# debbiemarkslab/EVcouplings

Measured on NVIDIA H100. Metric: PLM gradient evals/s as N*L^2*q cell-ops/s, higher is better.
Workload: dtype f32 parameters/accumulation; tensor-core products as bf16 hi+lo pairs (16 mantissa bits)

## Files before the change

evcouplings_b200/csrc/api.cu:

```cuda
#include "../../include/evcplm.h"

#include <stdlib.h>

#include <algorithm>
#include <new>
#include <string>
#include <vector>

#include "common.cuh"
#include "internal.h"

namespace evc {
static thread_local std::string g_err;
void set_error(const std::string &msg) { g_err = msg; }
}

using namespace evc;

static cudaStream_t as_stream(void *s) { return reinterpret_cast<cudaStream_t>(s); }

static const char SUPPORTED_Q[] =
    "supported: 2 <= q <= 32 states with the gap as a state, 2 <= q <= 31 with the ignored gap coded q; "
    "every code must be below 32, the 5 bit-planes of the Hamming pass";

// ... 392 lines not shown

int evc_plm_eval_data(evc_plm_t *h, const float *d_x, float *d_g, double *d_fx, void *stream)
{
    if (!h || !d_x || !d_g || !d_fx) { set_error("evc_plm_eval_data: null pointer"); return 1; }
    cudaStream_t st = as_stream(stream);
    const PlmGeom &g = h->g;
    const bool prof = h->profiling;
    const bool tc = h->bwd_mode == 1;
    const bool tcf = h->fwd_mode == 1;
    const bool tcff = h->fwd_mode == 2;
    const int single = h->precision == 1 ? 1 : 0;
    void *rt_lo = single ? nullptr : h->d_rt_lo;
    float *gJ = d_g + (int64_t)g.L * g.q;
    if (tc && h->tc.n_chunks > 1) {
        if (!tcf) {
            set_error("evc_plm_eval_data: sequence chunks need the tensor-core forward (evc_plm_set_forward 1)");
            return 1;
        }
        h->ev_valid = false;
        if (plm_tcf_expand(g, h->tcf, d_x, h->d_wt_hi, h->d_wt_lo, single, st)) return 1;
        for (int c = 0; c < h->tc.n_chunks; c++) {
            const int64_t n0 = (int64_t)c * h->tc.C, nreal = std::min(h->tc.C, g.N - n0);
            if (plm_tcf_build_xsp(g, h->tcf, h->d_msa4, h->d_x1h, n0, st)) return 1;
            if (plm_tc_build_xt(g, h->tc, h->d_msa4, h->d_xt, n0, st)) return 1;
            if (plm_tcf_logits(g, h->tcf, h->tcf_maps, h->d_x1h, h->d_zt, single, nreal, st)) return 1;
            if (plm_tcf_softmax(g, h->tcf, h->d_zt, d_x, h->d_msa4, h->d_wts, h->d_rt_hi, rt_lo, h->tc.Kp,
                                h->d_gh_part2, h->d_fx_part2, n0, nreal, st))
                return 1;
            if (plm_tc_backward(g, h->tc, h->tc_maps, h->d_Gd, single, c, st)) return 1;
        }
        if (plm_tc_finalize_pairs(g, h->tc, h->d_Gd, h->tc.planes, gJ, 1.0f, st)) return 1;
        return plm_finalize_fields_n(g, h->d_gh_part2, h->d_fx_part2, d_g, d_fx, h->tcf.ntiles_s, st);
    }
    if (!tc || (!tcf && !tcff)) {
        if (require_gather_q(h, "evc_plm_eval_data") || ensure_gather(h)) return 1;
    }
    if (prof) EVC_CUDA(cudaEventRecord(h->ev[0], st));
    if (tcff) {
        if (plm_tcff_expand(g, h->tcff, d_x, h->d_wp_hi, h->d_wp_lo, single, st)) return 1;
        if (prof) EVC_CUDA(cudaEventRecord(h->ev[1], st));
        if (plm_tcff_forward(g, h->tcff, h->tcff_maps, d_x, h->d_msa4, h->d_wts, h->d_rt_hi, h->d_rt_lo, h->tc.Kp,
                             h->d_gh_part3, h->d_fx_part3, single, st))
            return 1;
        if (prof) {
            EVC_CUDA(cudaEventRecord(h->ev[2], st));
            EVC_CUDA(cudaEventRecord(h->ev[3], st));
        }
// ... 45 lines not shown

int evc_plm_set_backward(evc_plm_t *h, int32_t mode)
{
    if (!h) { set_error("evc_plm_set_backward: null handle"); return 1; }
    if (mode != 0 && mode != 1) { set_error("evc_plm_set_backward: mode must be 0 (gather) or 1 (tensor core)"); return 1; }
    if (mode == 0 && require_gather_q(h, "evc_plm_set_backward")) return 1;
    EVC_CUDA(cudaSetDevice(h->device));
    if (mode == 1 && !h->d_xt) {
        int sm_count = 0;
        EVC_CUDA(cudaDeviceGetAttribute(&sm_count, cudaDevAttrMultiProcessorCount, h->device));
        plm_tc_geometry(h->g, sm_count, h->seq_chunk, h->tc);
        const PlmTcGeom &t = h->tc;
        const TcBwdBytes b(t);
        if (!dalloc(h, &h->d_xt, b.xt) || !dalloc(h, &h->d_rt_hi, b.rt) || !dalloc(h, &h->d_rt_lo, b.rt) ||
            !dalloc(h, &h->d_Gd, b.gd)) {
            set_error(std::string("evc_plm_set_backward: device allocation failed: ") +
                      cudaGetErrorString(cudaGetLastError()));
            return 1;
        }
        EVC_CUDA(cudaMemset(h->d_xt, 0, b.xt));
        EVC_CUDA(cudaMemset(h->d_rt_hi, 0, b.rt));
        EVC_CUDA(cudaMemset(h->d_rt_lo, 0, b.rt));
        EVC_CUDA(cudaMemset(h->d_Gd, 0, b.gd));
        if (t.n_chunks == 1 && plm_tc_build_xt(h->g, t, h->d_msa4, h->d_xt, 0, 0)) return 1;
        EVC_CUDA(cudaDeviceSynchronize());
        h->tc_maps = aligned_alloc(64, round_up((int64_t)plm_tc_map_bytes(), 64));
        if (!h->tc_maps) { set_error("evc_plm_set_backward: out of host memory"); return 1; }
        if (plm_tc_make_maps(t, h->d_xt, h->d_rt_hi, h->d_rt_lo, h->tc_maps)) return 1;
    }
    h->bwd_mode = mode;
    return 0;
}

int evc_plm_set_forward(evc_plm_t *h, int32_t mode)
{
    if (!h) { set_error("evc_plm_set_forward: null handle"); return 1; }
    if (mode < 0 || mode > 2) {
        set_error("evc_plm_set_forward: mode must be 0 (gather), 1 (tensor core) or 2 (tensor core, fused softmax)");
        return 1;
    }
    if (mode == 0 && require_gather_q(h, "evc_plm_set_forward")) return 1;
    EVC_CUDA(cudaSetDevice(h->device));
    const int64_t chunk = plm_seq_chunk_round(h->seq_chunk);
    const bool chunked = chunk > 0 && chunk < h->g.N;
    if (mode == 2 && (!plm_tcff_supported(h->g) || (int64_t)h->g.L * h->g.q > 8192 || chunked)) mode = 1;
    if (mode >= 1) {
        if (evc_plm_set_backward(h, 1)) return 1;
        if (!h->d_x1h) {
            plm_tcf_geometry(h->g, h->tc, h->tcf);
            const PlmTcfGeom &t = h->tcf;
            const TcFwdBytes b(h->g, t);
// ... 204 lines not shown
            set_error("evc_plm_eval_host: device allocation failed");
            return 1;
        }
    }
    EVC_CUDA(cudaMemcpyAsync(h->d_x_tmp, x, nb, cudaMemcpyHostToDevice, 0));
    if (evc_plm_eval_data(h, h->d_x_tmp, h->d_g_tmp, h->d_fx_tmp, nullptr)) return 1;
    if (evc_plm_add_regulariser(h, h->d_x_tmp, h->d_g_tmp, h->d_fx_tmp, lambda_h, lambda_J, nullptr)) return 1;
    EVC_CUDA(cudaMemcpyAsync(gout, h->d_g_tmp, nb, cudaMemcpyDeviceToHost, 0));
    EVC_CUDA(cudaMemcpyAsync(fx_out, h->d_fx_tmp, 2 * sizeof(double), cudaMemcpyDeviceToHost, 0));
    EVC_CUDA(cudaStreamSynchronize(0));
    return 0;
}

int evc_plm_weighted_counts(evc_plm_t *h, float *d_fi_counts, float *d_fij_counts, void *stream)
{
    if (!h || !d_fi_counts || !d_fij_counts) { set_error("evc_plm_weighted_counts: null pointer"); return 1; }
    cudaStream_t st = as_stream(stream);
    const PlmGeom &g = h->g;
    if (h->bwd_mode == 1 && h->d_gh_part2) {
        const int ntiles = h->tcf.ntiles_s;
        const PlmTcGeom &t = h->tc;
        for (int c = 0; c < t.n_chunks; c++) {
            const int64_t n0 = (int64_t)c * t.C, nreal = std::min(t.C, g.N - n0);
            if (t.n_chunks > 1 && plm_tc_build_xt(g, t, h->d_msa4, h->d_xt, n0, st)) return 1;
            if (plm_tc_onehot_residual(g, ntiles, h->d_msa4, h->d_wts, h->d_rt_hi, h->d_rt_lo, t.Kp, h->d_gh_part2,
                                       h->d_fx_part2, n0, nreal, st))
                return 1;
            if (plm_tc_backward(g, t, h->tc_maps, h->d_Gd, 0, c, st)) return 1;
        }
        if (plm_tc_finalize_pairs(g, t, h->d_Gd, t.planes, d_fij_counts, 0.5f, st)) return 1;
        return plm_finalize_fields_n(g, h->d_gh_part2, nullptr, d_fi_counts, nullptr, ntiles, st);
    }
    if (require_gather_q(h, "evc_plm_weighted_counts") || ensure_gather(h)) return 1;
    EVC_CUDA(cudaMemsetAsync(h->d_G, 0, (size_t)g.w_floats() * sizeof(float), st));
    if (plm_onehot_residual(g, h->d_msa4, h->d_wts, h->d_R, h->d_gh_part, st)) return 1;
    if (plm_backward(g, h->d_R, h->d_perm, h->d_bstart, h->d_G, st)) return 1;
    return plm_finalize(g, h->d_G, h->d_gh_part, nullptr, d_fi_counts, d_fij_counts, nullptr, 0.5f, st);
}

int evc_ec_scores(const float *d_J_tri, const float *d_fij_tri, const float *d_fi, int32_t L, int32_t q,
                  float *d_fn_raw, float *d_fn_zero_sum, float *d_mi, void *stream)
{
    if (!d_J_tri) { set_error("evc_ec_scores: null pointer"); return 1; }
    return ec_scores(d_J_tri, d_fij_tri, d_fi, L, q, d_fn_raw, d_fn_zero_sum, d_mi, as_stream(stream));
}

int evc_plm_energies(evc_plm_t *h, const float *d_x, double *d_out, void *stream)
// ... 75 lines not shown
```

evcouplings_b200/csrc/internal.h:

```cpp
#pragma once
#include <cuda_runtime.h>
#include <stdint.h>

namespace evc {

int64_t hamming_plane_words(int64_t N, int L);
int64_t hamming_num_tiles(int64_t N);
int hamming_pack(const uint8_t *d_codes, int64_t N, int L, uint32_t *d_planes, cudaStream_t st);
int hamming_count_tiles(const uint32_t *d_planes, const int *d_mult, int64_t N, int L, int min_identical,
                        int64_t tile_begin, int64_t tile_end, int *d_counts, cudaStream_t st);

int identities_to_seq(const uint8_t *d_codes, const uint8_t *d_seq, int64_t N, int L, int *d_out, cudaStream_t st);

int msa_unique(const uint8_t *d_codes, int64_t N, int L, int *d_first, int *d_inverse, int *d_mult, int64_t *U_out,
               cudaStream_t st);

struct PlmGeom {
    int64_t N;
    int L;
    int Lp;
    int q;
    int QB;
    int S;
    int gap_code;
// ... 29 lines not shown
                 float *d_G, cudaStream_t st);
int plm_finalize(const PlmGeom &g, const float *d_G, const float *d_gh_part, const double *d_fx_part,
                 float *d_gh, float *d_gJ, double *d_fx, float scale_pair, cudaStream_t st);

constexpr int64_t PLM_SEQ_CHUNK_ALIGN = 768;
int64_t plm_seq_chunk_round(int64_t seq_chunk);
struct PlmTcGeom {
    int64_t C;
    int n_chunks;
    int64_t Mp;
    int64_t Np;
    int64_t Kp;
    int ksplit;
    int ksplit_last;
    int planes;
    int64_t kp_chunk(int c, int64_t N) const
    {
        const int64_t n = N - (int64_t)c * C < C ? N - (int64_t)c * C : C;
        return (n + 63) / 64 * 64;
    }
};
void plm_tc_geometry(const PlmGeom &g, int sm_count, int64_t seq_chunk, PlmTcGeom &t);
size_t plm_tc_map_bytes();
int plm_tc_build_xt(const PlmGeom &g, const PlmTcGeom &t, const uint32_t *d_msa4, void *d_xt, int64_t n0,
                    cudaStream_t st);
int plm_tc_make_maps(const PlmTcGeom &t, void *d_xt, void *d_rt_hi, void *d_rt_lo, void *maps_out_host);
int plm_tc_backward(const PlmGeom &g, const PlmTcGeom &t, const void *maps_host, float *d_Gd, int single, int chunk,
                    cudaStream_t st);
int plm_tc_onehot_residual(const PlmGeom &g, int ntiles, const uint32_t *d_msa4, const float *d_wts, void *d_rt_hi,
                           void *d_rt_lo, int64_t Kp, float *d_gh_part, double *d_fx_part, int64_t n0, int64_t nreal,
                           cudaStream_t st);
int plm_tc_finalize_pairs(const PlmGeom &g, const PlmTcGeom &t, const float *d_Gd, int planes, float *d_gJ,
                          float scale, cudaStream_t st);
struct PlmTcfGeom {
    int64_t Mp;
    int64_t Kw;
    int64_t Ns;
    int64_t Xrows;
    int ntiles_s;
};
void plm_tcf_geometry(const PlmGeom &g, const PlmTcGeom &tc, PlmTcfGeom &t);
int plm_tcf_build_x(const PlmGeom &g, const PlmTcfGeom &t, const uint32_t *d_msa4, void *d_x1h, int64_t n0,
                    cudaStream_t st);
int plm_tcf_build_xsp(const PlmGeom &g, const PlmTcfGeom &t, const uint32_t *d_msa4, void *d_x1h, int64_t n0,
                      cudaStream_t st);
int plm_tcf_make_maps(const PlmTcfGeom &t, void *d_wt_hi, void *d_wt_lo, void *maps_out_host);
int plm_tcf_expand(const PlmGeom &g, const PlmTcfGeom &t, const float *d_x, void *d_wt_hi, void *d_wt_lo,
                   int single, cudaStream_t st);
int plm_tcf_logits(const PlmGeom &g, const PlmTcfGeom &t, const void *maps_host, const void *d_x1h, float *d_zt,
// ... 111 lines not shown
```

evcouplings_b200/csrc/plm_tc.cu:

```cuda
#include <cuda.h>
#include <cuda_bf16.h>

#include <stdlib.h>

#include <algorithm>

#include "common.cuh"
#include "internal.h"

namespace evc {

constexpr int TC_BM = 128;
constexpr int TC_BN = 192;
constexpr int TC_BK = 64;
constexpr int TC_MAX_STAGES = 8;
constexpr int TC_A_BYTES = TC_BM * TC_BK * 2;
constexpr int TC_B_BYTES = TC_BN * TC_BK * 2;
constexpr int TC_SMEM_LIMIT = 232448;
constexpr int TC_SMEM_HEAD = 2048;
constexpr int TC_THREADS = 384;
constexpr int TC_CONSUMERS = 256;
constexpr int TC_K_CHUNK = 32;
constexpr int TC_MAX_KSPLIT = 8;
constexpr int TC_REG_PRODUCER = 40;
// ... 59 lines not shown

template <int R>
__device__ __forceinline__ void fence_regs(float *d)
{
#pragma unroll
    for (int i = 0; i < R; i++) asm volatile("" : "+f"(d[i])::"memory");
}

__device__ __forceinline__ void consumer_sync() { asm volatile("bar.sync 1, %0;" ::"n"(TC_CONSUMERS) : "memory"); }

__device__ __forceinline__ uint64_t make_desc_sw128(const void *smem_ptr)
{
    const uint32_t addr = smem_u32(smem_ptr);
    uint64_t d = 0;
    d |= (uint64_t)((addr >> 4) & 0x3FFF);
    d |= (uint64_t)1 << 16;
    d |= (uint64_t)(1024 >> 4) << 32;
    d |= (uint64_t)1 << 62;
    return d;
}

template <int N>
__device__ __forceinline__ void wgmma_bf16(float *d, uint64_t da, uint64_t db, uint32_t scale_d);
template <>
__device__ __forceinline__ void wgmma_bf16<192>(float *d, uint64_t da, uint64_t db, uint32_t scale_d)
{
    asm volatile(
        "{\n.reg .pred p;\n"
        "setp.ne.b32 p, %98, 0;\n"
        "wgmma.mma_async.sync.aligned.m64n192k16.f32.bf16.bf16 "
        "{"
        "%0, %1, %2, %3, %4, %5, %6, %7, %8, %9, %10, %11, %12, %13, %14, %15, "
        "%16, %17, %18, %19, %20, %21, %22, %23, %24, %25, %26, %27, %28, %29, %30, %31, "
        "%32, %33, %34, %35, %36, %37, %38, %39, %40, %41, %42, %43, %44, %45, %46, %47, "
        "%48, %49, %50, %51, %52, %53, %54, %55, %56, %57, %58, %59, %60, %61, %62, %63, "
        "%64, %65, %66, %67, %68, %69, %70, %71, %72, %73, %74, %75, %76, %77, %78, %79, "
        "%80, %81, %82, %83, %84, %85, %86, %87, %88, %89, %90, %91, %92, %93, %94, %95"
        "}, %96, %97, p, 1, 1, 0, 0;\n}\n"
        : "+f"(d[0]), "+f"(d[1]), "+f"(d[2]), "+f"(d[3]), "+f"(d[4]), "+f"(d[5]), "+f"(d[6]), "+f"(d[7]),
          "+f"(d[8]), "+f"(d[9]), "+f"(d[10]), "+f"(d[11]), "+f"(d[12]), "+f"(d[13]), "+f"(d[14]), "+f"(d[15]),
          "+f"(d[16]), "+f"(d[17]), "+f"(d[18]), "+f"(d[19]), "+f"(d[20]), "+f"(d[21]), "+f"(d[22]), "+f"(d[23]),
          "+f"(d[24]), "+f"(d[25]), "+f"(d[26]), "+f"(d[27]), "+f"(d[28]), "+f"(d[29]), "+f"(d[30]), "+f"(d[31]),
          "+f"(d[32]), "+f"(d[33]), "+f"(d[34]), "+f"(d[35]), "+f"(d[36]), "+f"(d[37]), "+f"(d[38]), "+f"(d[39]),
          "+f"(d[40]), "+f"(d[41]), "+f"(d[42]), "+f"(d[43]), "+f"(d[44]), "+f"(d[45]), "+f"(d[46]), "+f"(d[47]),
          "+f"(d[48]), "+f"(d[49]), "+f"(d[50]), "+f"(d[51]), "+f"(d[52]), "+f"(d[53]), "+f"(d[54]), "+f"(d[55]),
          "+f"(d[56]), "+f"(d[57]), "+f"(d[58]), "+f"(d[59]), "+f"(d[60]), "+f"(d[61]), "+f"(d[62]), "+f"(d[63]),
          "+f"(d[64]), "+f"(d[65]), "+f"(d[66]), "+f"(d[67]), "+f"(d[68]), "+f"(d[69]), "+f"(d[70]), "+f"(d[71]),
          "+f"(d[72]), "+f"(d[73]), "+f"(d[74]), "+f"(d[75]), "+f"(d[76]), "+f"(d[77]), "+f"(d[78]), "+f"(d[79]),
          "+f"(d[80]), "+f"(d[81]), "+f"(d[82]), "+f"(d[83]), "+f"(d[84]), "+f"(d[85]), "+f"(d[86]), "+f"(d[87]),
          "+f"(d[88]), "+f"(d[89]), "+f"(d[90]), "+f"(d[91]), "+f"(d[92]), "+f"(d[93]), "+f"(d[94]), "+f"(d[95])
        : "l"(da), "l"(db), "r"(scale_d));
}
template <>
__device__ __forceinline__ void wgmma_bf16<176>(float *d, uint64_t da, uint64_t db, uint32_t scale_d)
{
    asm volatile(
        "{\n.reg .pred p;\n"
        "setp.ne.b32 p, %90, 0;\n"
        "wgmma.mma_async.sync.aligned.m64n176k16.f32.bf16.bf16 "
        "{"
        "%0, %1, %2, %3, %4, %5, %6, %7, %8, %9, %10, %11, %12, %13, %14, %15, "
        "%16, %17, %18, %19, %20, %21, %22, %23, %24, %25, %26, %27, %28, %29, %30, %31, "
        "%32, %33, %34, %35, %36, %37, %38, %39, %40, %41, %42, %43, %44, %45, %46, %47, "
        "%48, %49, %50, %51, %52, %53, %54, %55, %56, %57, %58, %59, %60, %61, %62, %63, "
        "%64, %65, %66, %67, %68, %69, %70, %71, %72, %73, %74, %75, %76, %77, %78, %79, "
        "%80, %81, %82, %83, %84, %85, %86, %87"
        "}, %88, %89, p, 1, 1, 0, 0;\n}\n"
        : "+f"(d[0]), "+f"(d[1]), "+f"(d[2]), "+f"(d[3]), "+f"(d[4]), "+f"(d[5]), "+f"(d[6]), "+f"(d[7]),
          "+f"(d[8]), "+f"(d[9]), "+f"(d[10]), "+f"(d[11]), "+f"(d[12]), "+f"(d[13]), "+f"(d[14]), "+f"(d[15]),
          "+f"(d[16]), "+f"(d[17]), "+f"(d[18]), "+f"(d[19]), "+f"(d[20]), "+f"(d[21]), "+f"(d[22]), "+f"(d[23]),
          "+f"(d[24]), "+f"(d[25]), "+f"(d[26]), "+f"(d[27]), "+f"(d[28]), "+f"(d[29]), "+f"(d[30]), "+f"(d[31]),
          "+f"(d[32]), "+f"(d[33]), "+f"(d[34]), "+f"(d[35]), "+f"(d[36]), "+f"(d[37]), "+f"(d[38]), "+f"(d[39]),
          "+f"(d[40]), "+f"(d[41]), "+f"(d[42]), "+f"(d[43]), "+f"(d[44]), "+f"(d[45]), "+f"(d[46]), "+f"(d[47]),
          "+f"(d[48]), "+f"(d[49]), "+f"(d[50]), "+f"(d[51]), "+f"(d[52]), "+f"(d[53]), "+f"(d[54]), "+f"(d[55]),
// ... 127 lines not shown
};
__device__ __forceinline__ TcSmem tc_smem_layout(unsigned char *smem_dyn)
{
    unsigned char *base = reinterpret_cast<unsigned char *>((reinterpret_cast<uintptr_t>(smem_dyn) + 1023) &
                                                            ~static_cast<uintptr_t>(1023));
    TcSmem l;
    l.full = reinterpret_cast<uint64_t *>(base);
    l.empty = l.full + TC_MAX_STAGES;
    l.ring = base + 1024;
    return l;
}
__device__ __forceinline__ void tc_init_barriers(const TcSmem &l, int n_stages)
{
    if (threadIdx.x == 0) {
        for (int s = 0; s < n_stages; s++) {
            mbar_init(&l.full[s], 1);
            mbar_init(&l.empty[s], TC_CONSUMERS);
        }
        mbar_fence_init();
    }
    __syncthreads();
}

template <int SINGLE, int ACC = 0>
__global__ void __launch_bounds__(TC_THREADS, 1)
tc_gemm_kernel(const __grid_constant__ CUtensorMap tm0, const __grid_constant__ CUtensorMap tm1,
               const __grid_constant__ CUtensorMap tm2, float *__restrict__ D, int64_t ldd, int m_tiles, int n_tiles,
               int num_kb, int k_chunk, int mgroup, int n_stages, int ksplit, int64_t plane, int acc_planes)
{
    constexpr int BYTES0 = TC_A_BYTES;
    constexpr int BYTES1 = TC_B_BYTES;
    constexpr int BYTES2 = TC_B_BYTES;
    constexpr int stage_bytes = BYTES0 + BYTES1 + (SINGLE ? 0 : BYTES2);
    extern __shared__ unsigned char smem_dyn[];
    const TcSmem l = tc_smem_layout(smem_dyn);
    const int tiles = m_tiles * n_tiles;
    const int slice = (int)blockIdx.x / tiles;
    int m_tile, n_tile;
    decode_tile((int)blockIdx.x - slice * tiles, m_tiles, n_tiles, mgroup, m_tile, n_tile);
    const int kb_per = (num_kb + ksplit - 1) / ksplit;
    const int kb_begin = slice * kb_per, kb_end = min(num_kb, kb_begin + kb_per);
    tc_init_barriers(l, n_stages);

    if (threadIdx.x < 128) {
        setmaxnreg_dec<TC_REG_PRODUCER>();
        if (threadIdx.x == 0) {
            int s = 0;
            uint32_t ph = 0;
            for (int kb = kb_begin; kb < kb_end; kb++) {
                mbar_wait_bounded(&l.empty[s], ph ^ 1u);
                unsigned char *st = l.ring + s * stage_bytes;
                mbar_expect_tx(&l.full[s], (uint32_t)stage_bytes);
                tma_load_2d(st, &tm0, kb * TC_BK, m_tile * TC_BM, &l.full[s]);
                tma_load_2d(st + BYTES0, &tm1, kb * TC_BK, n_tile * TC_BN, &l.full[s]);
                if (!SINGLE) tma_load_2d(st + BYTES0 + BYTES1, &tm2, kb * TC_BK, n_tile * TC_BN, &l.full[s]);
                if (++s == n_stages) { s = 0; ph ^= 1u; }
            }
        }
    } else {
        setmaxnreg_inc<TC_REG_CONSUMER>();
        const int cw = (threadIdx.x >> 7) - 1;
        constexpr uint64_t OFF1 = (uint64_t)(BYTES0 >> 4), OFF2 = (uint64_t)((BYTES0 + BYTES1) >> 4);
        const uint64_t arow = (uint64_t)((cw * 64 * TC_BK * 2) >> 4);
        const uint64_t desc0 = make_desc_sw128(l.ring);
        float acc[TC_BN / 2], sum[TC_BN / 2];
#pragma unroll
        for (int u = 0; u < TC_BN / 2; u++) acc[u] = 0.f;
        const int n_chunks = (kb_end - kb_begin + k_chunk - 1) / k_chunk;
        int s = 0;
        uint32_t ph = 0;
        for (int c = 0; c < n_chunks; c++) {
            const int kb0 = kb_begin + c * k_chunk, kb1 = min(kb_end, kb0 + k_chunk);
            tc_mainloop<TC_BN>(acc, l.full, l.empty, s, ph, n_stages, stage_bytes, kb0, kb1, desc0,
                               arow, OFF1, arow, OFF2, !SINGLE);
#pragma unroll
            for (int u = 0; u < TC_BN / 2; u++) sum[u] = (c == 0) ? acc[u] : sum[u] + acc[u];
        }
        const int t = threadIdx.x & 127;
        const int64_t row = (int64_t)m_tile * TC_BM + cw * 64 + (t >> 5) * 16 + ((t & 31) >> 2);
        float *out = D + slice * plane + row * ldd + (int64_t)n_tile * TC_BN + 2 * (t & 3);
        if (ACC && slice < acc_planes) {
#pragma unroll
            for (int c8 = 0; c8 < TC_BN / 8; c8++) {
                float2 *p0 = reinterpret_cast<float2 *>(out + 8 * c8);
                float2 *p1 = reinterpret_cast<float2 *>(out + 8 * ldd + 8 * c8);
                const float2 v0 = __ldcs(p0), v1 = __ldcs(p1);
                __stcs(p0, make_float2(v0.x + sum[4 * c8], v0.y + sum[4 * c8 + 1]));
                __stcs(p1, make_float2(v1.x + sum[4 * c8 + 2], v1.y + sum[4 * c8 + 3]));
            }
            return;
        }
#pragma unroll
        for (int c8 = 0; c8 < TC_BN / 8; c8++) {
            __stcs(reinterpret_cast<float2 *>(out + 8 * c8), make_float2(sum[4 * c8], sum[4 * c8 + 1]));
            __stcs(reinterpret_cast<float2 *>(out + 8 * ldd + 8 * c8), make_float2(sum[4 * c8 + 2], sum[4 * c8 + 3]));
        }
    }
}

constexpr int XSP_STEP_BYTES = 2560;
constexpr int XSP_KB_BYTES = 4 * XSP_STEP_BYTES;
constexpr int SP_W_HALF = (TC_BN / 2) * TC_BK * 2;

// ... 509 lines not shown
        if (n0 < N) {
            const int64_t off = ((int64_t)i * q + a) * Kp + nl;
            const __nv_bfloat162 hi = __floats2bfloat162_rn(z[0][a], z[1][a]);
            *reinterpret_cast<__nv_bfloat162 *>(Rt_hi + off) = hi;
            if (Rt_lo != nullptr)
                *reinterpret_cast<__nv_bfloat162 *>(Rt_lo + off) =
                    __floats2bfloat162_rn(z[0][a] - __low2float(hi), z[1][a] - __high2float(hi));
        }
        const float v = warp_sum(z[0][a] + z[1][a]);
        if (lane == 0) s_gh[warp * 32 + a] = v;
    }
    const double fw = warp_sum(fx_local);
    if (lane == 0) s_fx[warp] = fw;
    __syncthreads();
    if (tid < g.S) {
        float tot = 0.f;
        if (tid < q)
            for (int ww = 0; ww < 4; ww++) tot += s_gh[ww * 32 + tid];
        gh_part[((int64_t)i * ntiles + tile) * g.S + tid] = tot;
    }
    if (tid == 0) fx_part[(int64_t)i * ntiles + tile] = (s_fx[0] + s_fx[1]) + (s_fx[2] + s_fx[3]);
}

__global__ void build_xt_kernel(const uint32_t *__restrict__ msa4, __nv_bfloat16 *__restrict__ Xt, int64_t n0,
                                int64_t N, int64_t Nld, int64_t Kp, int L, int q)
{
    const int64_t n = (int64_t)blockIdx.x * blockDim.x + threadIdx.x;
    const int j = blockIdx.y;
    if (n >= Kp) return;
    int code = 255;
    if (n0 + n < N) code = (int)((msa4[(int64_t)(j >> 2) * Nld + n0 + n] >> (8 * (j & 3))) & 0xffu);
    for (int b = 0; b < q; b++)
        Xt[((int64_t)j * q + b) * Kp + n] = __float2bfloat16(code == b ? 1.0f : 0.0f);
}

constexpr int FIN_SITES = 4;
constexpr int FIN_W = FIN_SITES * 21;
constexpr int FIN_PITCH = FIN_W + 1;
constexpr int FIN_THREADS = 256;
constexpr int FIN_SMEM = 2 * FIN_W * FIN_PITCH * (int)sizeof(float);
constexpr int FIN_BATCH = 8;
static int fin_pitch(int q) { return q <= 21 ? FIN_PITCH : FIN_SITES * q + 1; }
static int fin_smem_bytes(int q) { return q <= 21 ? FIN_SMEM : 2 * (fin_pitch(q) - 1) * fin_pitch(q) * (int)sizeof(float); }

template <bool WIDE = false>
__global__ void __launch_bounds__(FIN_THREADS)
finalize_pairs_tc_kernel(const float *__restrict__ Gd, int planes, int64_t plane, float *__restrict__ gJ, int L,
                         int q, int Np, float scale, int wide_pitch)
{
    const int pitch = WIDE ? wide_pitch : FIN_PITCH;
    extern __shared__ float fin_smem[];
    float *sA = fin_smem;
    float *sB = fin_smem + (pitch - 1) * pitch;
    const int ti = blockIdx.y, tj = blockIdx.x;
    if (tj < ti) return;
    const int i0 = ti * FIN_SITES, j0 = tj * FIN_SITES;
// ... 65 lines not shown

static int stages_for(int stage_bytes)
{
    return std::max(2, std::min(TC_MAX_STAGES, (TC_SMEM_LIMIT - TC_SMEM_HEAD) / stage_bytes));
}

typedef CUresult (*PFN_encodeTiled)(CUtensorMap *, CUtensorMapDataType, cuuint32_t, void *, const cuuint64_t *,
                                    const cuuint64_t *, const cuuint32_t *, const cuuint32_t *, CUtensorMapInterleave,
                                    CUtensorMapSwizzle, CUtensorMapL2promotion, CUtensorMapFloatOOBfill);

static PFN_encodeTiled get_encode_fn()
{
    static PFN_encodeTiled fn = nullptr;
    if (fn) return fn;
    void *p = nullptr;
    cudaDriverEntryPointQueryResult qres;
    if (cudaGetDriverEntryPoint("cuTensorMapEncodeTiled", &p, cudaEnableDefault, &qres) != cudaSuccess ||
        qres != cudaDriverEntryPointSuccess || !p)
        return nullptr;
    fn = reinterpret_cast<PFN_encodeTiled>(p);
    return fn;
}

static int make_map(CUtensorMap *m, void *base, int64_t rows, int64_t kp, int box_rows)
{
    PFN_encodeTiled fn = get_encode_fn();
    if (!fn) { set_error("cuTensorMapEncodeTiled entry point not available"); return 1; }
    cuuint64_t gdim[2] = {(cuuint64_t)kp, (cuuint64_t)rows};
    cuuint64_t gstride[1] = {(cuuint64_t)kp * 2};
    cuuint32_t box[2] = {(cuuint32_t)TC_BK, (cuuint32_t)box_rows};
    cuuint32_t estr[2] = {1, 1};
    CUresult r = fn(m, CU_TENSOR_MAP_DATA_TYPE_BFLOAT16, 2, base, gdim, gstride, box, estr,
                    CU_TENSOR_MAP_INTERLEAVE_NONE, CU_TENSOR_MAP_SWIZZLE_128B, CU_TENSOR_MAP_L2_PROMOTION_L2_256B,
                    CU_TENSOR_MAP_FLOAT_OOB_FILL_NONE);
    if (r != CUDA_SUCCESS) { set_error("cuTensorMapEncodeTiled failed with code " + std::to_string((int)r)); return 1; }
    return 0;
}

static int backward_ksplit(int64_t tiles, int num_kb, int sm_count)
{
    static int ks_env = -2;
    const int e = env_int_once("EVC_KSPLIT", &ks_env);
    int ks = 1;
    if (e > 0) {
        ks = std::min(e, TC_MAX_KSPLIT);
    } else {
        double best = 0.0;
        for (int s = 1; s <= 4 && s <= num_kb; s++) {
            const int64_t units = tiles * s;
            const double eff = (double)units / ((double)sm_count * (double)ceil_div(units, sm_count));
            if (eff >= 0.97) { ks = s; break; }
            if (eff > best) { best = eff; ks = s; }
        }
    }
    ks = std::max(1, std::min(ks, num_kb));
    return (int)ceil_div(num_kb, ceil_div(num_kb, ks));
}

int64_t plm_seq_chunk_round(int64_t seq_chunk) { return seq_chunk <= 0 ? 0 : round_up(seq_chunk, PLM_SEQ_CHUNK_ALIGN); }

void plm_tc_geometry(const PlmGeom &g, int sm_count, int64_t seq_chunk, PlmTcGeom &t)
{
    const int64_t lq = (int64_t)g.L * g.q;
    const int64_t c = plm_seq_chunk_round(seq_chunk);
    t.C = (c == 0 || c >= g.N) ? g.N : c;
    t.n_chunks = (int)ceil_div(g.N, t.C);
    t.Mp = round_up(lq, TC_BM);
    t.Np = round_up(lq, TC_BN);
    t.Kp = round_up(t.C, TC_BK);
    const int64_t tiles = (t.Mp / TC_BM) * (t.Np / TC_BN);
    t.ksplit = backward_ksplit(tiles, (int)(t.Kp / TC_BK), sm_count);
    t.ksplit_last = backward_ksplit(tiles, (int)(t.kp_chunk(t.n_chunks - 1, g.N) / TC_BK), sm_count);
    t.planes = std::max(t.ksplit, t.ksplit_last);
}

int plm_tc_build_xt(const PlmGeom &g, const PlmTcGeom &t, const uint32_t *d_msa4, void *d_xt, int64_t n0,
                    cudaStream_t st)
{
    dim3 grid((unsigned)ceil_div(t.Kp, 256), (unsigned)g.L);
    build_xt_kernel<<<grid, 256, 0, st>>>(d_msa4, reinterpret_cast<__nv_bfloat16 *>(d_xt), n0, g.N, g.Nld, t.Kp,
                                          g.L, g.q);
    EVC_KERNEL_CHECK();
    return 0;
}

int plm_tc_make_maps(const PlmTcGeom &t, void *d_xt, void *d_rt_hi, void *d_rt_lo, void *maps_out)
{
    CUtensorMap *m = reinterpret_cast<CUtensorMap *>(maps_out);
    if (make_map(&m[0], d_xt, t.Mp, t.Kp, TC_BM)) return 1;
    if (make_map(&m[1], d_rt_hi, t.Np, t.Kp, TC_BN)) return 1;
    if (make_map(&m[2], d_rt_lo, t.Np, t.Kp, TC_BN)) return 1;
    return 0;
}

int plm_tc_backward(const PlmGeom &g, const PlmTcGeom &t, const void *maps, float *d_Gd, int single, int chunk,
                    cudaStream_t st)
{
    const CUtensorMap *m = reinterpret_cast<const CUtensorMap *>(maps);
    const int stage = TC_A_BYTES + TC_B_BYTES + (single ? 0 : TC_B_BYTES);
    const int n_stages = stages_for(stage);
    const size_t smem = (size_t)n_stages * stage + TC_SMEM_HEAD;
    static int kc_env = -2;
    const int kc = env_int_once("EVC_KCHUNK", &kc_env);
    const int k_chunk = kc > 0 ? kc : TC_K_CHUNK;
    const int m_tiles = (int)(t.Mp / TC_BM), n_tiles = (int)(t.Np / TC_BN);
    const bool last = chunk == t.n_chunks - 1;
    const int ksplit = last ? t.ksplit_last : t.ksplit;
    const int num_kb = (int)(t.kp_chunk(chunk, g.N) / TC_BK);
    const int grid = m_tiles * n_tiles * ksplit;
    const int64_t plane = t.Mp * t.Np;
    if (chunk == 0) {
        if (single) {
            EVC_CUDA(cudaFuncSetAttribute(tc_gemm_kernel<1>, cudaFuncAttributeMaxDynamicSharedMemorySize, TC_SMEM_LIMIT));
            tc_gemm_kernel<1><<<grid, TC_THREADS, smem, st>>>(m[0], m[1], m[2], d_Gd, t.Np, m_tiles, n_tiles,
                                                                num_kb, k_chunk, m_tiles, n_stages, ksplit, plane, 0);
        } else {
            EVC_CUDA(cudaFuncSetAttribute(tc_gemm_kernel<0>, cudaFuncAttributeMaxDynamicSharedMemorySize, TC_SMEM_LIMIT));
            tc_gemm_kernel<0><<<grid, TC_THREADS, smem, st>>>(m[0], m[1], m[2], d_Gd, t.Np, m_tiles, n_tiles,
                                                                num_kb, k_chunk, m_tiles, n_stages, ksplit, plane, 0);
        }
    } else {
        const int acc_planes = t.ksplit;
        if (single) {
            EVC_CUDA(cudaFuncSetAttribute(tc_gemm_kernel<1, 1>, cudaFuncAttributeMaxDynamicSharedMemorySize, TC_SMEM_LIMIT));
            tc_gemm_kernel<1, 1><<<grid, TC_THREADS, smem, st>>>(m[0], m[1], m[2], d_Gd, t.Np, m_tiles, n_tiles,
                                                                   num_kb, k_chunk, m_tiles, n_stages, ksplit, plane,
                                                                   acc_planes);
        } else {
            EVC_CUDA(cudaFuncSetAttribute(tc_gemm_kernel<0, 1>, cudaFuncAttributeMaxDynamicSharedMemorySize, TC_SMEM_LIMIT));
            tc_gemm_kernel<0, 1><<<grid, TC_THREADS, smem, st>>>(m[0], m[1], m[2], d_Gd, t.Np, m_tiles, n_tiles,
                                                                   num_kb, k_chunk, m_tiles, n_stages, ksplit, plane,
                                                                   acc_planes);
        }
    }
    EVC_KERNEL_CHECK();
    return 0;
}

int plm_tc_finalize_pairs(const PlmGeom &g, const PlmTcGeom &t, const float *d_Gd, int planes, float *d_gJ,
                          float scale, cudaStream_t st)
{
    const unsigned nt = (unsigned)ceil_div(g.L, FIN_SITES);
    auto kernel = g.q > 21 ? finalize_pairs_tc_kernel<true> : finalize_pairs_tc_kernel<false>;
    const int smem = fin_smem_bytes(g.q);
    EVC_CUDA(cudaFuncSetAttribute(kernel, cudaFuncAttributeMaxDynamicSharedMemorySize, smem));
    kernel<<<dim3(nt, nt), FIN_THREADS, smem, st>>>(d_Gd, planes, t.Mp * t.Np, d_gJ, g.L, g.q, (int)t.Np, scale,
                                                    fin_pitch(g.q));
    EVC_KERNEL_CHECK();
    return 0;
}

void plm_tcf_geometry(const PlmGeom &g, const PlmTcGeom &tc, PlmTcfGeom &t)
{
    const int64_t lq = (int64_t)g.L * g.q;
    t.Mp = round_up(lq, TC_BM);
    t.Kw = round_up(lq, TC_BK);
    t.Ns = round_up(tc.C, TC_BN);
// ... 212 lines not shown
```

Measured before the change: 5124 billion.

## Stream byte state codes to backward GEMM and expand one-hot A in registers

The backward tensor-core GEMM no longer reads a materialised bf16 one-hot X^T matrix of L*q rows. It TMA-loads one byte-code row per site and rebuilds the one-hot A fragments in registers with byte-compare bit tricks, feeding register-sourced wgmma (RS m64n192k16). This cuts A-operand global/L2 traffic and shared-memory footprint by roughly 2q, which allows more pipeline stages, and shrinks the build kernel. In exchange the consumer warps do extra ALU work per k-step, and the explicit software pipeline with wait<1> may expose more latency than the previous shared-memory-descriptor mainloop.

Result: faster. 5212 billion, median of 6 (+1.7%).

```diff
diff --git a/evcouplings_b200/csrc/api.cu b/evcouplings_b200/csrc/api.cu
--- a/evcouplings_b200/csrc/api.cu
+++ b/evcouplings_b200/csrc/api.cu
@@ -438,7 +438,7 @@
         for (int c = 0; c < h->tc.n_chunks; c++) {
             const int64_t n0 = (int64_t)c * h->tc.C, nreal = std::min(h->tc.C, g.N - n0);
             if (plm_tcf_build_xsp(g, h->tcf, h->d_msa4, h->d_x1h, n0, st)) return 1;
-            if (plm_tc_build_xt(g, h->tc, h->d_msa4, h->d_xt, n0, st)) return 1;
+            if (plm_tc_build_codes(g, h->tc, h->d_msa4, h->d_xt, n0, st)) return 1;
             if (plm_tcf_logits(g, h->tcf, h->tcf_maps, h->d_x1h, h->d_zt, single, nreal, st)) return 1;
             if (plm_tcf_softmax(g, h->tcf, h->d_zt, d_x, h->d_msa4, h->d_wts, h->d_rt_hi, rt_lo, h->tc.Kp,
                                 h->d_gh_part2, h->d_fx_part2, n0, nreal, st))
@@ -530,11 +530,11 @@
         EVC_CUDA(cudaMemset(h->d_rt_hi, 0, b.rt));
         EVC_CUDA(cudaMemset(h->d_rt_lo, 0, b.rt));
         EVC_CUDA(cudaMemset(h->d_Gd, 0, b.gd));
-        if (t.n_chunks == 1 && plm_tc_build_xt(h->g, t, h->d_msa4, h->d_xt, 0, 0)) return 1;
+        if (t.n_chunks == 1 && plm_tc_build_codes(h->g, t, h->d_msa4, h->d_xt, 0, 0)) return 1;
         EVC_CUDA(cudaDeviceSynchronize());
         h->tc_maps = aligned_alloc(64, round_up((int64_t)plm_tc_map_bytes(), 64));
         if (!h->tc_maps) { set_error("evc_plm_set_backward: out of host memory"); return 1; }
-        if (plm_tc_make_maps(t, h->d_xt, h->d_rt_hi, h->d_rt_lo, h->tc_maps)) return 1;
+        if (plm_tc_make_maps(h->g, t, h->d_xt, h->d_rt_hi, h->d_rt_lo, h->tc_maps)) return 1;
     }
     h->bwd_mode = mode;
     return 0;
@@ -785,7 +785,7 @@
         const PlmTcGeom &t = h->tc;
         for (int c = 0; c < t.n_chunks; c++) {
             const int64_t n0 = (int64_t)c * t.C, nreal = std::min(t.C, g.N - n0);
-            if (t.n_chunks > 1 && plm_tc_build_xt(g, t, h->d_msa4, h->d_xt, n0, st)) return 1;
+            if (t.n_chunks > 1 && plm_tc_build_codes(g, t, h->d_msa4, h->d_xt, n0, st)) return 1;
             if (plm_tc_onehot_residual(g, ntiles, h->d_msa4, h->d_wts, h->d_rt_hi, h->d_rt_lo, t.Kp, h->d_gh_part2,
                                        h->d_fx_part2, n0, nreal, st))
                 return 1;
diff --git a/evcouplings_b200/csrc/internal.h b/evcouplings_b200/csrc/internal.h
--- a/evcouplings_b200/csrc/internal.h
+++ b/evcouplings_b200/csrc/internal.h
@@ -75,9 +75,10 @@
 };
 void plm_tc_geometry(const PlmGeom &g, int sm_count, int64_t seq_chunk, PlmTcGeom &t);
 size_t plm_tc_map_bytes();
-int plm_tc_build_xt(const PlmGeom &g, const PlmTcGeom &t, const uint32_t *d_msa4, void *d_xt, int64_t n0,
-                    cudaStream_t st);
-int plm_tc_make_maps(const PlmTcGeom &t, void *d_xt, void *d_rt_hi, void *d_rt_lo, void *maps_out_host);
+int plm_tc_build_codes(const PlmGeom &g, const PlmTcGeom &t, const uint32_t *d_msa4, void *d_xt, int64_t n0,
+                       cudaStream_t st);
+int plm_tc_make_maps(const PlmGeom &g, const PlmTcGeom &t, void *d_xt, void *d_rt_hi, void *d_rt_lo,
+                     void *maps_out_host);
 int plm_tc_backward(const PlmGeom &g, const PlmTcGeom &t, const void *maps_host, float *d_Gd, int single, int chunk,
                     cudaStream_t st);
 int plm_tc_onehot_residual(const PlmGeom &g, int ntiles, const uint32_t *d_msa4, const float *d_wts, void *d_rt_hi,
diff --git a/evcouplings_b200/csrc/plm_tc.cu b/evcouplings_b200/csrc/plm_tc.cu
--- a/evcouplings_b200/csrc/plm_tc.cu
+++ b/evcouplings_b200/csrc/plm_tc.cu
@@ -105,12 +105,11 @@
 
 template <int N>
 __device__ __forceinline__ void wgmma_bf16(float *d, uint64_t da, uint64_t db, uint32_t scale_d);
-template <>
-__device__ __forceinline__ void wgmma_bf16<192>(float *d, uint64_t da, uint64_t db, uint32_t scale_d)
+__device__ __forceinline__ void wgmma_bf16_rs192(float *d, const uint32_t *a, uint64_t db, uint32_t scale_d)
 {
     asm volatile(
         "{\n.reg .pred p;\n"
-        "setp.ne.b32 p, %98, 0;\n"
+        "setp.ne.b32 p, %101, 0;\n"
         "wgmma.mma_async.sync.aligned.m64n192k16.f32.bf16.bf16 "
         "{"
         "%0, %1, %2, %3, %4, %5, %6, %7, %8, %9, %10, %11, %12, %13, %14, %15, "
@@ -119,7 +118,7 @@
         "%48, %49, %50, %51, %52, %53, %54, %55, %56, %57, %58, %59, %60, %61, %62, %63, "
         "%64, %65, %66, %67, %68, %69, %70, %71, %72, %73, %74, %75, %76, %77, %78, %79, "
         "%80, %81, %82, %83, %84, %85, %86, %87, %88, %89, %90, %91, %92, %93, %94, %95"
-        "}, %96, %97, p, 1, 1, 0, 0;\n}\n"
+        "}, {%96, %97, %98, %99}, %100, p, 1, 1, 0;\n}\n"
         : "+f"(d[0]), "+f"(d[1]), "+f"(d[2]), "+f"(d[3]), "+f"(d[4]), "+f"(d[5]), "+f"(d[6]), "+f"(d[7]),
           "+f"(d[8]), "+f"(d[9]), "+f"(d[10]), "+f"(d[11]), "+f"(d[12]), "+f"(d[13]), "+f"(d[14]), "+f"(d[15]),
           "+f"(d[16]), "+f"(d[17]), "+f"(d[18]), "+f"(d[19]), "+f"(d[20]), "+f"(d[21]), "+f"(d[22]), "+f"(d[23]),
@@ -132,7 +131,7 @@
           "+f"(d[72]), "+f"(d[73]), "+f"(d[74]), "+f"(d[75]), "+f"(d[76]), "+f"(d[77]), "+f"(d[78]), "+f"(d[79]),
           "+f"(d[80]), "+f"(d[81]), "+f"(d[82]), "+f"(d[83]), "+f"(d[84]), "+f"(d[85]), "+f"(d[86]), "+f"(d[87]),
           "+f"(d[88]), "+f"(d[89]), "+f"(d[90]), "+f"(d[91]), "+f"(d[92]), "+f"(d[93]), "+f"(d[94]), "+f"(d[95])
-        : "l"(da), "l"(db), "r"(scale_d));
+        : "r"(a[0]), "r"(a[1]), "r"(a[2]), "r"(a[3]), "l"(db), "r"(scale_d));
 }
 template <>
 __device__ __forceinline__ void wgmma_bf16<176>(float *d, uint64_t da, uint64_t db, uint32_t scale_d)
@@ -306,16 +305,41 @@
     __syncthreads();
 }
 
+constexpr uint32_t CODE_NONE = 0xFFu;
+__host__ __device__ constexpr int code_tile_bytes(int code_rows) { return (code_rows * TC_BK + 1023) & ~1023; }
+
+__device__ __forceinline__ uint32_t onehot_bytes(uint32_t w, uint32_t bb)
+{
+    const uint32_t x = w ^ bb;
+    return ~(((x & 0x7f7f7f7fu) + 0x7f7f7f7fu) | x) & 0x80808080u;
+}
+__device__ __forceinline__ void onehot_frag(uint32_t *a, uint32_t w0, uint32_t w1, uint32_t bb0, uint32_t bb1,
+                                            uint32_t mul0, uint32_t mul1)
+{
+    const uint32_t e0 = onehot_bytes(w0, bb0), e1 = onehot_bytes(w1, bb1);
+    a[0] = __byte_perm(e0, 0u, 0x4140) * mul0;
+    a[1] = __byte_perm(e1, 0u, 0x4140) * mul1;
+    a[2] = __byte_perm(e0, 0u, 0x4342) * mul0;
+    a[3] = __byte_perm(e1, 0u, 0x4342) * mul1;
+}
+
+__device__ __forceinline__ void fence_a(uint32_t *a)
+{
+#pragma unroll
+    for (int i = 0; i < 4; i++) asm volatile("" : "+r"(a[i])::"memory");
+}
+
 template <int SINGLE, int ACC = 0>
 __global__ void __launch_bounds__(TC_THREADS, 1)
 tc_gemm_kernel(const __grid_constant__ CUtensorMap tm0, const __grid_constant__ CUtensorMap tm1,
                const __grid_constant__ CUtensorMap tm2, float *__restrict__ D, int64_t ldd, int m_tiles, int n_tiles,
-               int num_kb, int k_chunk, int mgroup, int n_stages, int ksplit, int64_t plane, int acc_planes)
-{
-    constexpr int BYTES0 = TC_A_BYTES;
+               int num_kb, int k_chunk, int mgroup, int n_stages, int ksplit, int64_t plane, int acc_planes, int q,
+               int lq, int code_rows)
+{
     constexpr int BYTES1 = TC_B_BYTES;
     constexpr int BYTES2 = TC_B_BYTES;
-    constexpr int stage_bytes = BYTES0 + BYTES1 + (SINGLE ? 0 : BYTES2);
+    const int bytes0 = code_tile_bytes(code_rows);
+    const int stage_bytes = bytes0 + BYTES1 + (SINGLE ? 0 : BYTES2);
     extern __shared__ unsigned char smem_dyn[];
     const TcSmem l = tc_smem_layout(smem_dyn);
     const int tiles = m_tiles * n_tiles;
@@ -324,45 +348,89 @@
     decode_tile((int)blockIdx.x - slice * tiles, m_tiles, n_tiles, mgroup, m_tile, n_tile);
     const int kb_per = (num_kb + ksplit - 1) / ksplit;
     const int kb_begin = slice * kb_per, kb_end = min(num_kb, kb_begin + kb_per);
+    const int site0 = m_tile * TC_BM / q;
     tc_init_barriers(l, n_stages);
 
     if (threadIdx.x < 128) {
         setmaxnreg_dec<TC_REG_PRODUCER>();
         if (threadIdx.x == 0) {
+            const uint32_t tx = (uint32_t)(code_rows * TC_BK + BYTES1 + (SINGLE ? 0 : BYTES2));
             int s = 0;
             uint32_t ph = 0;
             for (int kb = kb_begin; kb < kb_end; kb++) {
                 mbar_wait_bounded(&l.empty[s], ph ^ 1u);
                 unsigned char *st = l.ring + s * stage_bytes;
-                mbar_expect_tx(&l.full[s], (uint32_t)stage_bytes);
-                tma_load_2d(st, &tm0, kb * TC_BK, m_tile * TC_BM, &l.full[s]);
-                tma_load_2d(st + BYTES0, &tm1, kb * TC_BK, n_tile * TC_BN, &l.full[s]);
-                if (!SINGLE) tma_load_2d(st + BYTES0 + BYTES1, &tm2, kb * TC_BK, n_tile * TC_BN, &l.full[s]);
+                mbar_expect_tx(&l.full[s], tx);
+                tma_load_2d(st, &tm0, kb * TC_BK, site0, &l.full[s]);
+                tma_load_2d(st + bytes0, &tm1, kb * TC_BK, n_tile * TC_BN, &l.full[s]);
+                if (!SINGLE) tma_load_2d(st + bytes0 + BYTES1, &tm2, kb * TC_BK, n_tile * TC_BN, &l.full[s]);
                 if (++s == n_stages) { s = 0; ph ^= 1u; }
             }
         }
     } else {
         setmaxnreg_inc<TC_REG_CONSUMER>();
         const int cw = (threadIdx.x >> 7) - 1;
-        constexpr uint64_t OFF1 = (uint64_t)(BYTES0 >> 4), OFF2 = (uint64_t)((BYTES0 + BYTES1) >> 4);
-        const uint64_t arow = (uint64_t)((cw * 64 * TC_BK * 2) >> 4);
-        const uint64_t desc0 = make_desc_sw128(l.ring);
+        const int t = threadIdx.x & 127;
+        const int row = m_tile * TC_BM + cw * 64 + (t >> 5) * 16 + ((t & 31) >> 2);
+        uint32_t off[2], bb[2], mask[2];
+#pragma unroll
+        for (int h = 0; h < 2; h++) {
+            const int m = row + 8 * h, j = m / q, b = m - j * q;
+            const bool live = m < lq;
+            off[h] = live ? (uint32_t)((j - site0) * TC_BK + 16 * (t & 3)) : 0xFFFFFFFFu;
+            bb[h] = (uint32_t)b * 0x01010101u;
+            mask[h] = live ? 0x7Fu : 0u;
+        }
+        auto code_word = [&](uint32_t stage_addr, int h, int k) -> uint32_t {
+            return off[h] == 0xFFFFFFFFu ? 0u : lds32(stage_addr + off[h] + 4 * k);
+        };
+        const uint32_t ring = smem_u32(l.ring);
+        const uint64_t desc0 = make_desc_sw128(l.ring + bytes0);
+        constexpr uint64_t OFF_LO = (uint64_t)(BYTES1 >> 4);
         float acc[TC_BN / 2], sum[TC_BN / 2];
+        uint32_t a[2][4];
 #pragma unroll
         for (int u = 0; u < TC_BN / 2; u++) acc[u] = 0.f;
+#pragma unroll
+        for (int i = 0; i < 4; i++) a[0][i] = a[1][i] = 0u;
         const int n_chunks = (kb_end - kb_begin + k_chunk - 1) / k_chunk;
         int s = 0;
         uint32_t ph = 0;
         for (int c = 0; c < n_chunks; c++) {
             const int kb0 = kb_begin + c * k_chunk, kb1 = min(kb_end, kb0 + k_chunk);
-            tc_mainloop<TC_BN>(acc, l.full, l.empty, s, ph, n_stages, stage_bytes, kb0, kb1, desc0,
-                               arow, OFF1, arow, OFF2, !SINGLE);
+            int prev = -1;
+            for (int kb = kb0; kb < kb1; kb++) {
+                mbar_wait_bounded(&l.full[s], ph);
+                const uint32_t sa = ring + (uint32_t)(s * stage_bytes);
+                const uint64_t d = desc0 + (uint64_t)((s * stage_bytes) >> 4);
+                uint32_t w0 = code_word(sa, 0, 0), w1 = code_word(sa, 1, 0);
+#pragma unroll
+                for (int k = 0; k < TC_BK / 16; k++) {
+                    uint32_t *ak = a[k & 1];
+                    onehot_frag(ak, w0, w1, bb[0], bb[1], mask[0], mask[1]);
+                    if (k + 1 < TC_BK / 16) { w0 = code_word(sa, 0, k + 1); w1 = code_word(sa, 1, k + 1); }
+                    const uint64_t koff = (uint64_t)((k * 16 * 2) >> 4);
+                    wgmma_fence();
+                    wgmma_bf16_rs192(acc, ak, d + koff, (kb == kb0 && k == 0) ? 0u : 1u);
+                    if (!SINGLE) wgmma_bf16_rs192(acc, ak, d + OFF_LO + koff, 1u);
+                    wgmma_commit();
+                    wgmma_wait<1>();
+                    fence_a(a[(k + 1) & 1]);
+                    if (k == 0 && prev >= 0) mbar_arrive(&l.empty[prev]);
+                }
+                prev = s;
+                if (++s == n_stages) { s = 0; ph ^= 1u; }
+            }
+            wgmma_wait<0>();
+            fence_regs<TC_BN / 2>(acc);
+            fence_a(a[0]);
+            fence_a(a[1]);
+            if (prev >= 0) mbar_arrive(&l.empty[prev]);
 #pragma unroll
             for (int u = 0; u < TC_BN / 2; u++) sum[u] = (c == 0) ? acc[u] : sum[u] + acc[u];
         }
-        const int t = threadIdx.x & 127;
-        const int64_t row = (int64_t)m_tile * TC_BM + cw * 64 + (t >> 5) * 16 + ((t & 31) >> 2);
-        float *out = D + slice * plane + row * ldd + (int64_t)n_tile * TC_BN + 2 * (t & 3);
+        const int64_t orow = row;
+        float *out = D + slice * plane + orow * ldd + (int64_t)n_tile * TC_BN + 2 * (t & 3);
         if (ACC && slice < acc_planes) {
 #pragma unroll
             for (int c8 = 0; c8 < TC_BN / 8; c8++) {
@@ -918,16 +986,23 @@
     if (tid == 0) fx_part[(int64_t)i * ntiles + tile] = (s_fx[0] + s_fx[1]) + (s_fx[2] + s_fx[3]);
 }
 
-__global__ void build_xt_kernel(const uint32_t *__restrict__ msa4, __nv_bfloat16 *__restrict__ Xt, int64_t n0,
-                                int64_t N, int64_t Nld, int64_t Kp, int L, int q)
-{
-    const int64_t n = (int64_t)blockIdx.x * blockDim.x + threadIdx.x;
+__global__ void build_codes_kernel(const uint32_t *__restrict__ msa4, uint32_t *__restrict__ codes, int64_t n0,
+                                   int64_t N, int64_t Nld, int64_t Kp, int q)
+{
+    const int64_t w = (int64_t)blockIdx.x * blockDim.x + threadIdx.x;
     const int j = blockIdx.y;
-    if (n >= Kp) return;
-    int code = 255;
-    if (n0 + n < N) code = (int)((msa4[(int64_t)(j >> 2) * Nld + n0 + n] >> (8 * (j & 3))) & 0xffu);
-    for (int b = 0; b < q; b++)
-        Xt[((int64_t)j * q + b) * Kp + n] = __float2bfloat16(code == b ? 1.0f : 0.0f);
+    if (w >= Kp / 4) return;
+    const int u = (int)(w >> 2) & 3, k = (int)w & 3;
+    const int64_t nb = n0 + (w >> 4) * TC_BK + 16 * k + 2 * u;
+    uint32_t v = 0;
+#pragma unroll
+    for (int e = 0; e < 4; e++) {
+        const int64_t n = nb + (e & 1) + 8 * (e >> 1);
+        uint32_t c = CODE_NONE;
+        if (n < N) c = (msa4[(int64_t)(j >> 2) * Nld + n] >> (8 * (j & 3))) & 0xffu;
+        v |= (c < (uint32_t)q ? c : CODE_NONE) << (8 * e);
+    }
+    codes[(int64_t)j * (Kp / 4) + w] = v;
 }
 
 constexpr int FIN_SITES = 4;
@@ -1039,19 +1114,24 @@
     return fn;
 }
 
-static int make_map(CUtensorMap *m, void *base, int64_t rows, int64_t kp, int box_rows)
+static int make_map_raw(CUtensorMap *m, CUtensorMapDataType type, int elem, void *base, int64_t rows, int64_t cols,
+                        int box_rows, CUtensorMapSwizzle swizzle)
 {
     PFN_encodeTiled fn = get_encode_fn();
     if (!fn) { set_error("cuTensorMapEncodeTiled entry point not available"); return 1; }
-    cuuint64_t gdim[2] = {(cuuint64_t)kp, (cuuint64_t)rows};
-    cuuint64_t gstride[1] = {(cuuint64_t)kp * 2};
+    cuuint64_t gdim[2] = {(cuuint64_t)cols, (cuuint64_t)rows};
+    cuuint64_t gstride[1] = {(cuuint64_t)cols * elem};
     cuuint32_t box[2] = {(cuuint32_t)TC_BK, (cuuint32_t)box_rows};
     cuuint32_t estr[2] = {1, 1};
-    CUresult r = fn(m, CU_TENSOR_MAP_DATA_TYPE_BFLOAT16, 2, base, gdim, gstride, box, estr,
-                    CU_TENSOR_MAP_INTERLEAVE_NONE, CU_TENSOR_MAP_SWIZZLE_128B, CU_TENSOR_MAP_L2_PROMOTION_L2_256B,
-                    CU_TENSOR_MAP_FLOAT_OOB_FILL_NONE);
+    CUresult r = fn(m, type, 2, base, gdim, gstride, box, estr, CU_TENSOR_MAP_INTERLEAVE_NONE, swizzle,
+                    CU_TENSOR_MAP_L2_PROMOTION_L2_256B, CU_TENSOR_MAP_FLOAT_OOB_FILL_NONE);
     if (r != CUDA_SUCCESS) { set_error("cuTensorMapEncodeTiled failed with code " + std::to_string((int)r)); return 1; }
     return 0;
+}
+
+static int make_map(CUtensorMap *m, void *base, int64_t rows, int64_t kp, int box_rows)
+{
+    return make_map_raw(m, CU_TENSOR_MAP_DATA_TYPE_BFLOAT16, 2, base, rows, kp, box_rows, CU_TENSOR_MAP_SWIZZLE_128B);
 }
 
 static int backward_ksplit(int64_t tiles, int num_kb, int sm_count)
@@ -1091,20 +1171,30 @@
     t.planes = std::max(t.ksplit, t.ksplit_last);
 }
 
-int plm_tc_build_xt(const PlmGeom &g, const PlmTcGeom &t, const uint32_t *d_msa4, void *d_xt, int64_t n0,
-                    cudaStream_t st)
-{
-    dim3 grid((unsigned)ceil_div(t.Kp, 256), (unsigned)g.L);
-    build_xt_kernel<<<grid, 256, 0, st>>>(d_msa4, reinterpret_cast<__nv_bfloat16 *>(d_xt), n0, g.N, g.Nld, t.Kp,
-                                          g.L, g.q);
+static int code_rows(const PlmGeom &g, const PlmTcGeom &t)
+{
+    const int64_t lq = (int64_t)g.L * g.q;
+    int r = 1;
+    for (int64_t m0 = 0; m0 < t.Mp && m0 < lq; m0 += TC_BM)
+        r = std::max(r, (int)(std::min(m0 + TC_BM, lq) - 1) / g.q - (int)(m0 / g.q) + 1);
+    return r;
+}
+
+int plm_tc_build_codes(const PlmGeom &g, const PlmTcGeom &t, const uint32_t *d_msa4, void *d_xt, int64_t n0,
+                       cudaStream_t st)
+{
+    dim3 grid((unsigned)ceil_div(t.Kp / 4, 256), (unsigned)g.L);
+    build_codes_kernel<<<grid, 256, 0, st>>>(d_msa4, reinterpret_cast<uint32_t *>(d_xt), n0, g.N, g.Nld, t.Kp, g.q);
     EVC_KERNEL_CHECK();
     return 0;
 }
 
-int plm_tc_make_maps(const PlmTcGeom &t, void *d_xt, void *d_rt_hi, void *d_rt_lo, void *maps_out)
+int plm_tc_make_maps(const PlmGeom &g, const PlmTcGeom &t, void *d_xt, void *d_rt_hi, void *d_rt_lo, void *maps_out)
 {
     CUtensorMap *m = reinterpret_cast<CUtensorMap *>(maps_out);
-    if (make_map(&m[0], d_xt, t.Mp, t.Kp, TC_BM)) return 1;
+    if (make_map_raw(&m[0], CU_TENSOR_MAP_DATA_TYPE_UINT8, 1, d_xt, g.L, t.Kp, code_rows(g, t),
+                     CU_TENSOR_MAP_SWIZZLE_NONE))
+        return 1;
     if (make_map(&m[1], d_rt_hi, t.Np, t.Kp, TC_BN)) return 1;
     if (make_map(&m[2], d_rt_lo, t.Np, t.Kp, TC_BN)) return 1;
     return 0;
@@ -1114,7 +1204,8 @@
                     cudaStream_t st)
 {
     const CUtensorMap *m = reinterpret_cast<const CUtensorMap *>(maps);
-    const int stage = TC_A_BYTES + TC_B_BYTES + (single ? 0 : TC_B_BYTES);
+    const int rows = code_rows(g, t);
+    const int stage = code_tile_bytes(rows) + TC_B_BYTES + (single ? 0 : TC_B_BYTES);
     const int n_stages = stages_for(stage);
     const size_t smem = (size_t)n_stages * stage + TC_SMEM_HEAD;
     static int kc_env = -2;
@@ -1126,30 +1217,13 @@
     const int num_kb = (int)(t.kp_chunk(chunk, g.N) / TC_BK);
     const int grid = m_tiles * n_tiles * ksplit;
     const int64_t plane = t.Mp * t.Np;
-    if (chunk == 0) {
-        if (single) {
-            EVC_CUDA(cudaFuncSetAttribute(tc_gemm_kernel<1>, cudaFuncAttributeMaxDynamicSharedMemorySize, TC_SMEM_LIMIT));
-            tc_gemm_kernel<1><<<grid, TC_THREADS, smem, st>>>(m[0], m[1], m[2], d_Gd, t.Np, m_tiles, n_tiles,
-                                                                num_kb, k_chunk, m_tiles, n_stages, ksplit, plane, 0);
-        } else {
-            EVC_CUDA(cudaFuncSetAttribute(tc_gemm_kernel<0>, cudaFuncAttributeMaxDynamicSharedMemorySize, TC_SMEM_LIMIT));
-            tc_gemm_kernel<0><<<grid, TC_THREADS, smem, st>>>(m[0], m[1], m[2], d_Gd, t.Np, m_tiles, n_tiles,
-                                                                num_kb, k_chunk, m_tiles, n_stages, ksplit, plane, 0);
-        }
-    } else {
-        const int acc_planes = t.ksplit;
-        if (single) {
-            EVC_CUDA(cudaFuncSetAttribute(tc_gemm_kernel<1, 1>, cudaFuncAttributeMaxDynamicSharedMemorySize, TC_SMEM_LIMIT));
-            tc_gemm_kernel<1, 1><<<grid, TC_THREADS, smem, st>>>(m[0], m[1], m[2], d_Gd, t.Np, m_tiles, n_tiles,
-                                                                   num_kb, k_chunk, m_tiles, n_stages, ksplit, plane,
-                                                                   acc_planes);
-        } else {
-            EVC_CUDA(cudaFuncSetAttribute(tc_gemm_kernel<0, 1>, cudaFuncAttributeMaxDynamicSharedMemorySize, TC_SMEM_LIMIT));
-            tc_gemm_kernel<0, 1><<<grid, TC_THREADS, smem, st>>>(m[0], m[1], m[2], d_Gd, t.Np, m_tiles, n_tiles,
-                                                                   num_kb, k_chunk, m_tiles, n_stages, ksplit, plane,
-                                                                   acc_planes);
-        }
-    }
+    const int acc_planes = t.ksplit;
+    auto kernel = chunk == 0 ? (single ? tc_gemm_kernel<1> : tc_gemm_kernel<0>)
+                             : (single ? tc_gemm_kernel<1, 1> : tc_gemm_kernel<0, 1>);
+    EVC_CUDA(cudaFuncSetAttribute(kernel, cudaFuncAttributeMaxDynamicSharedMemorySize, TC_SMEM_LIMIT));
+    kernel<<<grid, TC_THREADS, smem, st>>>(m[0], m[1], m[2], d_Gd, t.Np, m_tiles, n_tiles, num_kb, k_chunk, m_tiles,
+                                           n_stages, ksplit, plane, chunk == 0 ? 0 : acc_planes, g.q, g.L * g.q,
+                                           rows);
     EVC_KERNEL_CHECK();
     return 0;
 }
```
